# NikolausDemmel/rootba

Measured on NVIDIA H100. Metric: ms/LM-iter (linearize+QR+PCG) on BAL at 1/2/4/8 H100 vs CPU ref, lower is better.
Workload: dtype f32

## Files before the change

rootba_b200/csrc/kernels.cuh:

```cuda
#pragma once

#include <cooperative_groups.h>
#include <cuda_runtime.h>

#include <cfloat>
#include <cmath>
#include <cstdint>

#include "layout.hpp"

namespace rba {

template <class S> struct ST;
template <> struct ST<float> {
  using V2 = float2;
  using V4 = float4;
  __host__ __device__ static float eps_sqrt() { return 0.0031622776601683794f; }
  __host__ __device__ static float eps() { return 1e-5f; }
  __host__ __device__ static float tiny() { return FLT_MIN; }
};
template <> struct ST<double> {
  using V2 = double2;
  using V4 = double4;
  __host__ __device__ static double eps_sqrt() { return 1e-5; }
  __host__ __device__ static double eps() { return 1e-10; }
  __host__ __device__ static double tiny() { return DBL_MIN; }
};

__device__ __forceinline__ float2 mk2(float a, float b) { return make_float2(a, b); }
__device__ __forceinline__ double2 mk2(double a, double b) { return make_double2(a, b); }

struct KOpts {
  int use_valid_projections_only;
  int robust_norm;
  double huber;
  double jacobi_eps;
  int write_panel;
};

struct PcgState {
  double rho[2];
  double q0[2];
  double norm_b;
  double last_pq, last_alpha, last_zeta;
  int iter;
  int done;
  int term;
  int reason;
};

constexpr int NPART = 64;

template <class S>
struct DevPtrs {
  S* cams; S* lms;
  const TileInfo* tiles; int ntiles;
  const int* sorted_lm;
  const int* slot_cam; const int* slot_lm; const S* slot_xy; int nslots;
  S* panel;
  S* jp;
  S* q1u;
  S* q1d;
  S* jl;
  S* res;
  S* lmk;
  S* qtr;
  S* dmp;
  S* blk0;
  S* diag2; S* scaling; S* b; S* x; S* r; S* z; S* p; S* q; S* y; S* inc;
  S* blocks;
  S* jblocks;
  S* blocks0;
  S* b0;
  S* inv;
  S* yobs;
  S* partial;
  S* pblk;
  int nc;
  const uint8_t* cam_fixed;
  const S* prior_H;
  const int* pair_ptr;
  const int* pair_nbr;
  const S* pair_O;
  S* pair_ov;
  const int* lmp_slot;
  const S* lmp_mean;
  const S* lmp_L;
  S* lmp_Lg;
  const S* obs_W;
};
// ... 875 lines not shown
        V2* pk = ptile + (size_t)k * 32 + lane;
        const S nw00 = vc[0] ? -w0[0] : S(0), nw01 = vc[0] ? -w1[0] : S(0), nw02 = vc[0] ? -w2[0] : S(0);
        const S nw10 = vc[1] ? -w0[1] : S(0), nw11 = vc[1] ? -w1[1] : S(0), nw12 = vc[1] ? -w2[1] : S(0);
        const S* vp = sV + 9;
#pragma unroll 4
        for (int r = 3; r < nrows; ++r, vp += 3) {
          const S v0 = vp[0], v1 = vp[1], v2 = vp[2];
          pk[(size_t)(r - 3) * KP * 32] = mk2(nw00 * v0 + nw01 * v1 + nw02 * v2, nw10 * v0 + nw11 * v1 + nw12 * v2);
        }
#pragma unroll
        for (int v = 0; v < 2; ++v) {
          if (!vc[v]) continue;
#pragma unroll
          for (int q = 0; q < 2; ++q) {
            const int r = r2i[v] + q;
            if (r >= 3) {
              const S* vq = sV + 3 * r;
              const S val = (q == 0 ? a0[v] : a1[v]) - (w0[v] * vq[0] + w1[v] * vq[1] + w2[v] * vq[2]);
              S* dst = reinterpret_cast<S*>(pk + (size_t)(r - 3) * KP * 32) + v;
              *dst = val;
            }
          }
        }
      }
    }
#undef A_AT
    for (int e = lane; e < Wn; e += 32) sQ[28 * e + 27] = 0;
    __syncwarp();
    warp_copy_out(D.q1u + 28 * (size_t)T.slot_base, sQ, T.nvalid * n * 28, lane);
    __syncwarp();
  }
}


__host__ __device__ inline int stage2_need(int n, int G, int KP) {
  const int W = 32 / G, Wn = W * n;
  const int CS = (2 * G * KP) | 1;
  return 3 * W * CS + Wn * 9 + W * 20 + 8;
}

template <class S>
__device__ __forceinline__ void lm_prior_compress(const S* __restrict__ Lg, S sl, S (&C)[3][3], S (&c)[3]) {
  S M[6][4];
#pragma unroll
  for (int r = 0; r < 3; ++r) {
#pragma unroll
    for (int k = 0; k < 3; ++k) { M[r][k] = Lg[3 * r + k]; M[3 + r][k] = r == k ? sl : S(0); }
    M[r][3] = Lg[9 + r];
    M[3 + r][3] = 0;
  }
#pragma unroll
  for (int k = 0; k < 3; ++k)
#pragma unroll
    for (int m = k + 1; m < 6; ++m) {
      const Rot<S> gq = make_givens(M[k][k], M[m][k]);
#pragma unroll
      for (int cc = k; cc < 4; ++cc) rot_apply(gq, M[m][cc], M[k][cc]);
    }
#pragma unroll
  for (int r = 0; r < 3; ++r) {
#pragma unroll
    for (int k = 0; k < 3; ++k) C[r][k] = k >= r ? M[r][k] : S(0);
    c[r] = M[r][3];
  }
}

template <class S, bool PANEL, bool LMP = false>
__global__ void __launch_bounds__(128) k_stage2(DevPtrs<S> D, S lambda, Scratch<S> sc, int write_panel) {
  extern __shared__ __align__(16) unsigned char smem_raw[];
  using V2 = typename ST<S>::V2;
  const int wib = threadIdx.x >> 5, lane = threadIdx.x & 31;
  S* ws_smem = reinterpret_cast<S*>(smem_raw) + (size_t)wib * sc.smem_cap;
  for (int t = blockIdx.x * (blockDim.x >> 5) + wib; t < D.ntiles; t += gridDim.x * (blockDim.x >> 5)) {
    const TileInfo T = D.tiles[t];
    const int n = T.n, G = T.G, KP = T.KP, W = 32 / G, Wn = W * n;
    const int ncols = 9 * n;
    const int CS = (2 * G * KP) | 1;
    const int g = lane / G, j = lane - g * G;
    const bool active = g < T.nvalid;
    S* ws = scratch_ptr(sc, ws_smem, stage2_need(n, G, KP));
    S* sD = ws;
    S* sG = sD + 3 * W * CS;
    S* sRot = sG + Wn * 9;
    if (lane < T.nvalid) {
      S* lk = D.lmk + 24 * (size_t)(T.lm_base + lane);
      S Rw[3][3] = {{lk[0], lk[1], lk[2]}, {0, lk[3], lk[4]}, {0, 0, lk[5]}};
      S Dw[3][3] = {{0, 0, 0}, {0, 0, 0}, {0, 0, 0}};
      S rr[3] = {lk[6], lk[7], lk[8]}, dr[3] = {0, 0, 0};
      S* ro = sRot + 20 * lane;
      int lp = -1;
      if constexpr (LMP) lp = D.lmp_slot[T.lm_base + lane];
      if (lambda == S(0) && lp < 0) {
#pragma unroll
        for (int q = 0; q < 6; ++q) { ro[2 * q] = 1; ro[2 * q + 1] = 0; }
      } else {
        const S sl = sqrt(lambda);
        if (LMP && lp >= 0) lm_prior_compress(D.lmp_Lg + 12 * (size_t)lp, sl, Dw, dr);
        else { Dw[0][0] = sl; Dw[1][1] = sl; Dw[2][2] = sl; }
        int q = 0;
#pragma unroll
        for (int nn = 0; nn < 3; ++nn)
#pragma unroll
          for (int m = 0; m <= nn; ++m) {
            const int d = nn - m;
            const Rot<S> gq = make_givens(Rw[nn][nn], Dw[d][nn]);
            ro[2 * q] = gq.c; ro[2 * q + 1] = gq.s;
            ++q;
#pragma unroll
            for (int c = 0; c < 3; ++c) rot_apply(gq, Dw[d][c], Rw[nn][c]);
            rot_apply(gq, dr[d], rr[nn]);
          }
      }
      ro[12] = rr[0]; ro[13] = rr[1]; ro[14] = rr[2];
      ro[15] = dr[0]; ro[16] = dr[1]; ro[17] = dr[2];
      lk[9] = Rw[0][0]; lk[10] = Rw[0][1]; lk[11] = Rw[0][2]; lk[12] = Rw[1][1]; lk[13] = Rw[1][2]; lk[14] = Rw[2][2];
      lk[15] = rr[0]; lk[16] = rr[1]; lk[17] = rr[2];
    }
    __syncwarp();
    if (active) {
      Rot<S> rot[6];
      const S* ro = sRot + 20 * g;
#pragma unroll
      for (int q = 0; q < 6; ++q) { rot[q].c = ro[2 * q]; rot[q].s = ro[2 * q + 1]; }
      const S rr0 = ro[12], rr1 = ro[13], rr2 = ro[14];
      const S dr0 = ro[15], dr1 = ro[16], dr2 = ro[17];
      for (int i = j; i < n; i += G) {
        const size_t sl = (size_t)(T.slot_base + g * n + i);
        S q[28], jp[PANEL ? 4 : 20], dm[PANEL ? 28 : 4];
        load_rec<S, 28>(D.q1u + 28 * sl, q);
        S r0 = 0, r1 = 0;
        if constexpr (!PANEL) {
          load_rec<S, 20>(D.jp + 20 * sl, jp);
          r0 = D.res[2 * sl]; r1 = D.res[2 * sl + 1];
        }
        S* d0 = sD + (0 * W + g) * CS + 9 * i;
        S* d1 = sD + (1 * W + g) * CS + 9 * i;
        S* d2 = sD + (2 * W + g) * CS + 9 * i;
        S* go = sG + 9 * (g * n + i);
#pragma unroll
        for (int p = 0; p < 9; ++p) {
          S qv[3] = {q[p], q[9 + p], q[18 + p]}, dv[3] = {0, 0, 0};
          int qi = 0;
#pragma unroll
          for (int nn = 0; nn < 3; ++nn)
#pragma unroll
            for (int m = 0; m <= nn; ++m) rot_apply(rot[qi++], dv[nn - m], qv[nn]);
          q[p] = qv[0]; q[9 + p] = qv[1]; q[18 + p] = qv[2];
          d0[p] = dv[0]; d1[p] = dv[1]; d2[p] = dv[2];
          if constexpr (PANEL) {
            dm[p] = dv[0]; dm[9 + p] = dv[1]; dm[18 + p] = dv[2];
            go[p] = dv[0] * dr0 + dv[1] * dr1 + dv[2] * dr2;
          } else {
            go[p] = jp[p] * r0 + jp[9 + p] * r1 - (qv[0] * rr0 + qv[1] * rr1 + qv[2] * rr2);
          }
        }
        q[27] = 0;
        store_rec<S, 28>(D.q1d + 28 * sl, q);
        if constexpr (PANEL) {
          dm[27] = 0;
          store_rec<S, 28>(D.dmp + 28 * sl, dm);
        }
      }
    }
    __syncwarp();
    {
      const int nsl = T.nvalid * n;
      for (int e = lane; e < nsl * 9; e += 32) D.yobs[9 * (size_t)T.slot_base + e] = sG[e];
      if constexpr (!PANEL) {
        if (D.dmp)
          for (int e = lane; e < nsl * 28; e += 32) {
            const int sl = e / 28, k = e - 28 * sl, gg = sl / n, d = k / 9;
            D.dmp[28 * (size_t)T.slot_base + e] = k < 27 ? sD[(d * W + gg) * CS + 9 * (sl - gg * n) + (k - 9 * d)] : S(0);
          }
      }
      if (active && write_panel) {
        V2* ptile = reinterpret_cast<V2*>(D.panel + T.panel_off) + (size_t)(2 * n - 3) * KP * 32 + lane;
        for (int k = 0; k < KP; ++k) {
          const int c = 2 * j + 2 * G * k;
#pragma unroll
          for (int d = 0; d < 3; ++d) {
            const S* row = sD + (d * W + g) * CS;
            ptile[((size_t)d * KP + k) * 32] = mk2(c < ncols ? row[c] : S(0), c + 1 < ncols ? row[c + 1] : S(0));
          }
        }
      }
    }
    __syncwarp();
  }
}

template <class S, bool LMP = false>
__global__ void __launch_bounds__(128) k_sc_stage2(DevPtrs<S> D, S lambda) {
  const int wib = threadIdx.x >> 5, lane = threadIdx.x & 31;
  for (int t = blockIdx.x * (blockDim.x >> 5) + wib; t < D.ntiles; t += gridDim.x * (blockDim.x >> 5)) {
    const TileInfo T = D.tiles[t];
    const int n = T.n, G = T.G;
    const int g = lane / G, j = lane - g * G;
    const bool active = g < T.nvalid;
    const size_t slot0 = (size_t)(T.slot_base + g * n);
    S h[6] = {0, 0, 0, 0, 0, 0}, gv[3] = {0, 0, 0};
    if (active) {
      for (int i = j; i < n; i += G) {
        const S* jl = D.jl + 6 * (slot0 + i);
        const S r0 = D.res[2 * (slot0 + i)], r1 = D.res[2 * (slot0 + i) + 1];
        const S a0 = jl[0], a1 = jl[1], a2 = jl[2], b0 = jl[3], b1 = jl[4], b2 = jl[5];
        h[0] += a0 * a0 + b0 * b0; h[1] += a0 * a1 + b0 * b1; h[2] += a0 * a2 + b0 * b2;
        h[3] += a1 * a1 + b1 * b1; h[4] += a1 * a2 + b1 * b2; h[5] += a2 * a2 + b2 * b2;
        gv[0] += a0 * r0 + b0 * r1; gv[1] += a1 * r0 + b1 * r1; gv[2] += a2 * r0 + b2 * r1;
      }
    }
#pragma unroll
    for (int k = 0; k < 6; ++k) h[k] = group_sum(h[k], G);
#pragma unroll
    for (int k = 0; k < 3; ++k) gv[k] = group_sum(gv[k], G);
    if constexpr (LMP) {
      const int lp = D.lmp_slot[T.lm_base + g];
      if (lp >= 0) {
        const S* pg = D.lmp_Lg + 12 * (size_t)lp;
#pragma unroll
        for (int r = 0; r < 3; ++r) {
          const S a0 = pg[3 * r], a1 = pg[3 * r + 1], a2 = pg[3 * r + 2], gr = pg[9 + r];
          h[0] += a0 * a0; h[1] += a0 * a1; h[2] += a0 * a2; h[3] += a1 * a1; h[4] += a1 * a2; h[5] += a2 * a2;
          gv[0] += a0 * gr; gv[1] += a1 * gr; gv[2] += a2 * gr;
        }
      }
    }
    h[0] += lambda; h[3] += lambda; h[5] += lambda;
    const S r00 = sqrt(h[0]);
    const S r01 = h[1] / r00, r02 = h[2] / r00;
    const S r11 = sqrt(h[3] - r01 * r01);
    const S r12 = (h[4] - r01 * r02) / r11;
    const S r22 = sqrt(h[5] - r02 * r02 - r12 * r12);
    const S rr0 = gv[0] / r00;
    const S rr1 = (gv[1] - r01 * rr0) / r11;
    const S rr2 = (gv[2] - r02 * rr0 - r12 * rr1) / r22;
    if (active && j == 0) {
      S* lk = D.lmk + 24 * (size_t)(T.lm_base + g);
      lk[9] = r00; lk[10] = r01; lk[11] = r02; lk[12] = r11; lk[13] = r12; lk[14] = r22;
      lk[15] = rr0; lk[16] = rr1; lk[17] = rr2;
    }
    if (active) {
      for (int i = j; i < n; i += G) {
        const size_t sl = slot0 + i;
        S jp[20], q[28];
        load_rec<S, 20>(D.jp + 20 * sl, jp);
        const S* jl = D.jl + 6 * sl;
        const S a0 = jl[0], a1 = jl[1], a2 = jl[2], b0 = jl[3], b1 = jl[4], b2 = jl[5];
        const S r0 = D.res[2 * sl], r1 = D.res[2 * sl + 1];
        S* go = D.yobs + 9 * sl;
#pragma unroll
        for (int p = 0; p < 9; ++p) {
          const S t0 = a0 * jp[p] + b0 * jp[9 + p], t1 = a1 * jp[p] + b1 * jp[9 + p], t2 = a2 * jp[p] + b2 * jp[9 + p];
          const S c0 = t0 / r00;
          const S c1 = (t1 - r01 * c0) / r11;
          const S c2 = (t2 - r02 * c0 - r12 * c1) / r22;
          q[p] = c0; q[9 + p] = c1; q[18 + p] = c2;
          go[p] = jp[p] * r0 + jp[9 + p] * r1 - (c0 * rr0 + c1 * rr1 + c2 * rr2);
        }
        q[27] = 0;
        store_rec<S, 28>(D.q1d + 28 * sl, q);
      }
    }
  }
}

template <class S>
__global__ void __launch_bounds__(128) k_matvec_implicit(DevPtrs<S> D, int tile_begin, const S* __restrict__ xvec, const int* done, int pdl,
                                                          int e0_only = 0) {
  if (done && *reinterpret_cast<const volatile int*>(done)) return;
  if (pdl) asm volatile("griddepcontrol.wait;" ::: "memory");
  if (done && *done) return;
  if (pdl) asm volatile("griddepcontrol.launch_dependents;" ::: "memory");
  const int wib = threadIdx.x >> 5, lane = threadIdx.x & 31;
  for (int t = tile_begin + blockIdx.x * (blockDim.x >> 5) + wib; t < D.ntiles; t += gridDim.x * (blockDim.x >> 5)) {
    const TileInfo T = D.tiles[t];
    const int n = T.n, G = T.G;
    const int g = lane / G, j = lane - g * G;
    const bool active = g < T.nvalid;
    const size_t sl0 = (size_t)(T.slot_base + g * n);
    S u0 = 0, u1 = 0, u2 = 0;
    if (active) {
      for (int i = j; i < n; i += G) {
        const size_t sl = sl0 + i;
        S q[28];
        load_rec<S, 28>(D.q1d + 28 * sl, q);
        const S* xc = xvec + 9 * (size_t)D.slot_cam[sl];
#pragma unroll
        for (int p = 0; p < 9; ++p) {
          const S xv = xc[p];
          u0 += q[p] * xv; u1 += q[9 + p] * xv; u2 += q[18 + p] * xv;
        }
      }
    }
    u0 = group_sum(u0, G); u1 = group_sum(u1, G); u2 = group_sum(u2, G);
    if (active) {
      for (int i = j; i < n; i += G) {
        const size_t sl = sl0 + i;
        S q[28], jp[20];
        load_rec<S, 28>(D.q1d + 28 * sl, q);
        load_rec<S, 20>(D.jp + 20 * sl, jp);
        const S* xc = xvec + 9 * (size_t)D.slot_cam[sl];
        S t0 = 0, t1 = 0;
#pragma unroll
        for (int p = 0; p < 9; ++p) {
          const S xv = xc[p];
          t0 += jp[p] * xv; t1 += jp[9 + p] * xv;
        }
        S* yo = D.yobs + 9 * sl;
#pragma unroll
        for (int p = 0; p < 9; ++p) {
          const S e0 = q[p] * u0 + q[9 + p] * u1 + q[18 + p] * u2;
          yo[p] = e0_only ? e0 : (jp[p] * t0 + jp[9 + p] * t1) - e0;
        }
      }
    }
  }
}

template <class S, int MODE>
__global__ void __launch_bounds__(128) k_precond_partial(const S* __restrict__ recA, const S* __restrict__ recB,
                                                          const int* __restrict__ slots, const ReduceItem* __restrict__ items,
                                                          int nitems, S* __restrict__ pblk) {
  const int it = blockIdx.x * blockDim.x + threadIdx.x;
  if (it >= nitems) return;
  const ReduceItem I = items[it];
  S acc[45];
#pragma unroll
  for (int k = 0; k < 45; ++k) acc[k] = 0;
  for (int e = I.begin; e < I.end; ++e) {
    const size_t sl = (size_t)slots[e];
    if constexpr (MODE == 3) {
      S v[48];
      load_rec<S, 48>(recA + 48 * sl, v);
#pragma unroll
      for (int k = 0; k < 45; ++k) acc[k] += v[k];
    } else if constexpr (MODE == 2) {
      S v[28];
      load_rec<S, 28>(recA + 28 * sl, v);
      int k = 0;
#pragma unroll
      for (int a = 0; a < 9; ++a)
#pragma unroll
        for (int b = a; b < 9; ++b) acc[k++] += v[a] * v[b] + v[9 + a] * v[9 + b] + v[18 + a] * v[18 + b];
    } else {
      S v[20], w[MODE == 1 ? 28 : 4];
      load_rec<S, 20>(recA + 20 * sl, v);
      if constexpr (MODE == 1) load_rec<S, 28>(recB + 28 * sl, w);
      int k = 0;
#pragma unroll
      for (int a = 0; a < 9; ++a)
#pragma unroll
        for (int b = a; b < 9; ++b) {
          S sacc = v[a] * v[b] + v[9 + a] * v[9 + b];
          if constexpr (MODE == 1) sacc -= w[a] * w[b] + w[9 + a] * w[9 + b] + w[18 + a] * w[18 + b];
          acc[k++] += sacc;
        }
    }
  }
  S* o = pblk + 48 * (size_t)it;
#pragma unroll
  for (int k = 0; k < 45; ++k) o[k] = acc[k];
}

template <class S>
__global__ void k_precond_final(const S* __restrict__ pblk, const int* __restrict__ cam_item_ptr, int nc,
                                const S* __restrict__ addend, S* __restrict__ blocks) {
  const int i = blockIdx.x * blockDim.x + threadIdx.x;
  if (i >= 45 * nc) return;
  const int cam = i / 45, k = i - 45 * cam;
  S s = 0;
  for (int it = cam_item_ptr[cam]; it < cam_item_ptr[cam + 1]; ++it) s += pblk[48 * (size_t)it + k];
  int a = 0, rem = k;
  while (rem >= 9 - a) { rem -= 9 - a; ++a; }
  const int b = a + rem;
  if (addend) s += addend[81 * (size_t)cam + 9 * a + b];
  blocks[81 * (size_t)cam + 9 * a + b] = s;
  blocks[81 * (size_t)cam + 9 * b + a] = s;
}

template <class S>
__global__ void __launch_bounds__(128) k_panel_grad_blocks(DevPtrs<S> D, int want_blocks, TileOrder to) {
  using V2 = typename ST<S>::V2;
  const int wib = threadIdx.x >> 5, lane = threadIdx.x & 31;
  for (int idx = blockIdx.x * (blockDim.x >> 5) + wib;; idx += gridDim.x * (blockDim.x >> 5)) {
    const int t = tile_at(to, idx, D.ntiles);
    if (t < 0) break;
    const TileInfo T = D.tiles[t];
    const int n = T.n, G = T.G, KP = T.KP;
    const int lg = 31 - __clz(G);
    const int nobs = T.nvalid * n;
    const int nrows = 2 * n - 3;
    const V2* __restrict__ ptile = reinterpret_cast<const V2*>(D.panel + T.panel_off);
    const size_t rstride = (size_t)KP * 32;
    for (int e = lane; e < nobs; e += 32) {
      const int g = e / n, i = e - g * n;
      const int c0 = 9 * i;
      const bool odd = c0 & 1;
      const int p0 = c0 >> 1;
      int off[5];
#pragma unroll
      for (int q = 0; q < 5; ++q) {
        const int p = p0 + q;
        off[q] = (p >> lg) * 32 + g * G + (p & (G - 1));
      }
      const S* __restrict__ tq = D.qtr + 2 * (size_t)(T.slot_base + g * n) + 3;
      S acc[45], gacc[9];
#pragma unroll
      for (int k = 0; k < 45; ++k) acc[k] = 0;
#pragma unroll
      for (int k = 0; k < 9; ++k) gacc[k] = 0;
#pragma unroll 2
      for (int r = 0; r < nrows; ++r) {
        const V2* pr = ptile + (size_t)r * rstride;
        V2 a[5];
#pragma unroll
        for (int q = 0; q < 5; ++q) a[q] = __ldg(pr + off[q]);
        const S tr = __ldg(tq + r);
        const S el[10] = {a[0].x, a[0].y, a[1].x, a[1].y, a[2].x, a[2].y, a[3].x, a[3].y, a[4].x, a[4].y};
        S v[9];
#pragma unroll
        for (int k = 0; k < 9; ++k) v[k] = odd ? el[k + 1] : el[k];
#pragma unroll
        for (int k = 0; k < 9; ++k) gacc[k] += v[k] * tr;
        if (want_blocks) {
          int k = 0;
#pragma unroll
          for (int x = 0; x < 9; ++x)
#pragma unroll
            for (int y = x; y < 9; ++y) acc[k++] += v[x] * v[y];
        }
      }
      const size_t sl = (size_t)(T.slot_base + e);
#pragma unroll
      for (int k = 0; k < 9; ++k) D.yobs[9 * sl + k] = gacc[k];
      if (want_blocks) {
        S o[48];
#pragma unroll
        for (int k = 0; k < 45; ++k) o[k] = acc[k];
        o[45] = o[46] = o[47] = 0;
        store_rec<S, 48>(D.blk0 + 48 * sl, o);
      }
    }
  }
}

template <class S>
__global__ void __launch_bounds__(64) k_precond_invert(const S* __restrict__ src, S lambda, int nc,
                                                        S* __restrict__ blocks_out, S* __restrict__ inv,
                                                        const uint8_t* __restrict__ cam_fixed, S* __restrict__ b,
                                                        const S* __restrict__ prior_H = nullptr, const S* __restrict__ prior_g = nullptr) {
  const int cam = blockIdx.x * blockDim.x + threadIdx.x;
  if (cam >= nc) return;
  const unsigned fm = cam_fixed ? fixed_entry_mask(cam_fixed[cam]) : 0u;
  S A[9][9];
#pragma unroll
  for (int r = 0; r < 9; ++r)
#pragma unroll
    for (int c = 0; c < 9; ++c) A[r][c] = src[81 * (size_t)cam + 9 * r + c];
  if (prior_H)
#pragma unroll
    for (int r = 0; r < 9; ++r)
#pragma unroll
      for (int c = 0; c < 9; ++c) A[r][c] += prior_H[81 * (size_t)cam + 9 * r + c];
  if (prior_g)
#pragma unroll
    for (int d = 0; d < 9; ++d) b[9 * (size_t)cam + d] += prior_g[9 * (size_t)cam + d];
#pragma unroll
  for (int d = 0; d < 9; ++d) A[d][d] += lambda;
  if (blocks_out)
#pragma unroll
    for (int r = 0; r < 9; ++r)
#pragma unroll
      for (int c = 0; c < 9; ++c) blocks_out[81 * (size_t)cam + 9 * r + c] = A[r][c];
  if (fm) {
#pragma unroll
    for (int r = 0; r < 9; ++r)
#pragma unroll
      for (int c = 0; c < 9; ++c)
        if (((fm >> r) | (fm >> c)) & 1u) A[r][c] = (r == c) ? S(1) : S(0);
#pragma unroll
    for (int d = 0; d < 9; ++d)
      if ((fm >> d) & 1u) b[9 * (size_t)cam + d] = S(0);
  }
#pragma unroll
  for (int jj = 0; jj < 9; ++jj) {
    S sdiag = A[jj][jj];
#pragma unroll
    for (int k = 0; k < jj; ++k) sdiag -= A[jj][k] * A[jj][k];
    const S d = sqrt(sdiag);
    A[jj][jj] = d;
#pragma unroll
    for (int i = jj + 1; i < 9; ++i) {
      S t = A[jj][i];
#pragma unroll
      for (int k = 0; k < jj; ++k) t -= A[i][k] * A[jj][k];
      A[i][jj] = t / d;
    }
  }
  S Li[9][9];
#pragma unroll
  for (int c = 0; c < 9; ++c) {
#pragma unroll
    for (int r = 0; r < 9; ++r) {
      if (r < c) Li[r][c] = 0;
      else {
        S t = (r == c) ? S(1) : S(0);
#pragma unroll
        for (int k = 0; k < 9; ++k) if (k >= c && k < r) t -= A[r][k] * Li[k][c];
        Li[r][c] = t / A[r][r];
      }
    }
  }
  if (fm)
#pragma unroll
    for (int d = 0; d < 9; ++d)
      if ((fm >> d) & 1u) Li[d][d] = S(0);
  S* out = inv + 81 * (size_t)cam;
#pragma unroll
  for (int r = 0; r < 9; ++r)
#pragma unroll
    for (int c = r; c < 9; ++c) {
      S t = 0;
#pragma unroll
      for (int k = 0; k < 9; ++k) if (k >= c) t += Li[k][r] * Li[k][c];
// ... 1469 lines not shown
```

rootba_b200/csrc/solver.cu:

```cuda
#include <cuda_runtime.h>
#include <dlfcn.h>

#include <cstdio>
#include <cstdlib>
#include <cstring>
#include <chrono>
#include <array>
#include <limits>
#include <memory>
#include <string>
#include <utility>
#include <vector>

#include "../../include/rootba_b200.h"
#include "../host/bal_io_fast.hpp"
#include "kernels.cuh"
#include "covariance.cuh"
#include "assembled.cuh"
#include "groups.cuh"
#include "nccl_dyn.hpp"

namespace rba {

thread_local std::string g_err;
// ... 1027 lines not shown
  int compute_error(rba_residual_info* out) override {
    int rc = compute_error_enqueue(); if (rc) return rc;
    if (error_enqueued) CU(cudaStreamSynchronize(stream));
    return compute_error_finish(out);
  }

  int linearize_enqueue() {
    lin_l0 = launches;
    const int n_pairs = pprior.n, n_groups = grp.n;
    int rc = start(ev_stage1); if (rc) return rc;
    CU(cudaMemsetAsync(d_flags, 0, 4 * sizeof(int), stream));
    auto kn = D.obs_W ? k_jp_norms<S, true> : k_jp_norms<S>;
    kn<<<grid_for(L.nslots, 256, 8), 256, 0, stream>>>(D, ko, d_flags);
    ++launches;
    rc = camera_reduce(d_csr_obs_slots, d_csr_obs_items, n_obs_items, d_csr_obs_item_ptr, D.diag2); if (rc) return rc;
    if (cprior.on) {
      k_prior_linearize<S><<<(nc + 127) / 128, 128, 0, stream>>>(D.cams, cprior.mean.get(), cprior.L.get(), nc, D.diag2, cprior.A.get(), cprior.r.get());
      ++launches;
    }
    if (n_pairs > 0) {
      k_pair_linearize<S><<<(n_pairs + 127) / 128, 128, 0, stream>>>(D.cams, pprior.ij.get(), pprior.mean.get(), pprior.L.get(), n_pairs, pprior.A.get(), pprior.r.get());
      k_pair_diag2<S><<<(nc + 127) / 128, 128, 0, stream>>>(pprior.A.get(), pprior.ptr.get(), pprior.item.get(), nc, D.diag2);
      launches += 2;
    }
    if (n_groups) {
      k_group_sum_diag2<S><<<n_groups, GROUP_THREADS, 0, stream>>>(D.diag2, groups());
      ++launches;
    }
    k_scaling<S><<<(9 * nc + 255) / 256, 256, 0, stream>>>(D.diag2, D.scaling, 9 * nc, (S)ko.jacobi_eps);
    const bool lmp = D.lmp_slot != nullptr;
    auto k1 = opt.use_householder_marginalization ? (lmp ? k_linearize_qr<S, false, true> : k_linearize_qr<S, false>)
                                                  : (lmp ? k_linearize_qr<S, true, true> : k_linearize_qr<S, true>);
    if (D.obs_W)
      k1 = opt.use_householder_marginalization ? (lmp ? k_linearize_qr<S, false, true, true> : k_linearize_qr<S, false, false, true>)
                                               : (lmp ? k_linearize_qr<S, true, true, true> : k_linearize_qr<S, true, false, true>);
    k1<<<tile_grid(k1_max_blocks), TILE_WARPS * 32, k1_smem, stream>>>(D, ko, k1_sc, d_flags, order_k1);
    launches += 2;
    if (opt.preconditioner_type == 0 || opt.solver_type == 2) {
      rc = precond_blocks(0, D.jblocks, nullptr, true); if (rc) return rc;
    }
    const bool jac = opt.preconditioner_type == 0 || opt.solver_type == 2;
    if (cprior.on) {
      k_prior_scale<S><<<(nc + 127) / 128, 128, 0, stream>>>(cprior.A.get(), cprior.r.get(), D.scaling, nc, cprior.H.get(), cprior.g.get(), jac ? D.jblocks : nullptr);
      ++launches;
    }
    if (n_pairs > 0) {
      k_pair_scale<S><<<(n_pairs + 127) / 128, 128, 0, stream>>>(pprior.A.get(), pprior.ij.get(), D.scaling, n_pairs);
      k_pair_accum<S><<<(nc + 127) / 128, 128, 0, stream>>>(pprior.A.get(), pprior.r.get(), pprior.ptr.get(), pprior.item.get(), nc, (int)cprior.on,
                                                            cprior.H.get(), cprior.g.get(), jac ? D.jblocks : nullptr, pprior.O.get());
      launches += 2;
    }
    if (panel_form()) {
      const int want_blocks = opt.preconditioner_type == 1 ? 1 : 0;
      k_panel_grad_blocks<S><<<tile_grid(sm_count * 8), TILE_WARPS * 32, 0, stream>>>(D, want_blocks, order_kp);
      ++launches;
      rc = camera_reduce(d_csr_obs_slots, d_csr_obs_items, n_obs_items, d_csr_obs_item_ptr, D.b0, nullptr, false); if (rc) return rc;
      if (want_blocks) { rc = precond_blocks(3, D.blocks0, nullptr, false); if (rc) return rc; }
    }
    rc = allreduce_scalars(0); if (rc) return rc;
    CU(cudaMemcpyAsync(h_res->linearize_flags, d_flags, sizeof(h_res->linearize_flags), cudaMemcpyDeviceToHost, stream));
    rc = stop(ev_stage1); if (rc) return rc;
    linearized = true;
    new_linearization_point = true;
    su_valid = s_valid = false;
    damping_valid = false;
    have_inc = false;
    return RBA_OK;
  }
  int linearize_finish() {
    CU(cudaGetLastError());
    tm.stage1_time = elapsed(ev_stage1);
    tm.kernel_launches = launches - lin_l0;
    if (h_res->linearize_flags[1]) { linearized = false; g_err = "a peer rank did not take part in a cross-shard reduction in time (peer-memory exchange timed out)"; return RBA_ERR_NCCL; }
    if (h_res->linearize_flags[0]) { linearized = false; return RBA_NUMERICAL_FAILURE; }
    return RBA_OK;
  }
  int linearize() override {
    int rc = linearize_enqueue(); if (rc) return rc;
    CU(cudaStreamSynchronize(stream));
    return linearize_finish();
  }

  int precond_blocks(int mode, S* dst, const S* addend, bool reduce_ranks) {
    const int g = (n_pb_items + 127) / 128;
    switch (mode) {
      case 0: k_precond_partial<S, 0><<<g, 128, 0, stream>>>(D.jp, (const S*)nullptr, d_csr_obs_slots, d_pb_items, n_pb_items, D.pblk); break;
      case 1: k_precond_partial<S, 1><<<g, 128, 0, stream>>>(D.jp, D.q1d, d_csr_obs_slots, d_pb_items, n_pb_items, D.pblk); break;
      case 2: k_precond_partial<S, 2><<<g, 128, 0, stream>>>(D.dmp, (const S*)nullptr, d_csr_obs_slots, d_pb_items, n_pb_items, D.pblk); break;
      default: k_precond_partial<S, 3><<<g, 128, 0, stream>>>(D.blk0, (const S*)nullptr, d_csr_obs_slots, d_pb_items, n_pb_items, D.pblk); break;
    }
    k_precond_final<S><<<(45 * nc + 255) / 256, 256, 0, stream>>>(D.pblk, d_pb_item_ptr, nc, addend, dst);
    launches += 2;
    return reduce_ranks ? allreduce(dst, (size_t)81 * nc) : RBA_OK;
  }

  enum class Handover {
    Assembled,
    Partials,
    Counter,
    Peer,
    Nccl,
  };
  Handover handover() const {
    if (s_valid) return Handover::Assembled;
    if (grp.n) return opt.nranks > 1 ? Handover::Nccl : Handover::Counter;
    if (opt.nranks > 1) return peer_ok ? Handover::Peer : Handover::Nccl;
    const bool vec_cached = 9 * ((nc + pcg_cluster - 1) / pcg_cluster) <= VEC_THREADS * VEC_EPT;
    return pcg_partials && vec_cached && opt.solver_type != 2 ? Handover::Partials : Handover::Counter;
  }
  int apply_operator(const S* xvec, Handover h, bool in_solve, int e0_only = 0) {
    const int* done = in_solve ? &d_state->done : nullptr;
    const bool pdl = in_solve;
    ++tm.matvec_launches;
    if (h == Handover::Assembled) {
      const bool p = pdl && !s_fresh;
      s_fresh = false;
      return launch_ex(k_rcs_spmv<S>, spmv_grid, SPMV_CLASSES * 32, 0, p, 1, (const SpmvChunk*)d_spmv_chunks, (const int*)d_spmv_chunk_ptr,
                       (const int*)d_asm_col, (const S*)d_asm_S, xvec, D.y, done, (int)p);
    }
    if (panels) {
      if (L.n_items_large > 0) {
        k_matvec_large<S, K4_WARPS, KPMAX><<<grid_for(L.n_items_large, K4_WARPS, 4), K4_WARPS * 32, k4_smem_small, stream>>>(
            D, d_items, 0, L.n_items_large, L.k4_scratch_per_warp, xvec, done);
        ++launches;
      }
      const bool p = pdl && L.n_items_large == 0;
      if (n_dealt > L.n_items_large)
        TRY(launch_ex(k_matvec_small_tma<S, K4_WARPS, K4_NS, K4_STAGE>, tma_grid, K4_WARPS * 32, K4_SMEM_TMA, p, 1, D, (const MatvecItem*)d_items, L.n_items_large, n_dealt, xvec, done, (int)p));
    } else {
      const int ntl = (int)L.tiles.size();
      const bool p = pdl && imp_tile_split == ntl;
      if (imp_tile_split > 0)
        TRY(launch_ex((k_matvec_implicit_tma<S, IMP_WARPS, IMP_MAXSLOTS, IMP_NS>), imp_grid, IMP_WARPS * 32, imp_smem, p, 1, D, imp_tile_split, xvec, done, (int)p, e0_only));
      if (imp_tile_split < ntl)
        TRY(launch_ex(k_matvec_implicit<S>, (ntl - imp_tile_split + TILE_WARPS - 1) / TILE_WARPS, TILE_WARPS * 32, 0, false, 1, D, imp_tile_split, xvec, done, 0, e0_only));
    }
    const int grid = grid_for(n_op_items, 8, 8);
    if (h == Handover::Partials)
      return launch_ex(k_cam_reduce<S>, grid, 256, 0, pdl, 1, (const S*)D.yobs, op_slots, op_items, n_op_items, D.partial, done, (int)pdl);
    if (h == Handover::Peer) ++ar_seq;
    if (h == Handover::Nccl) CU(cudaMemsetAsync(D.y, 0, (size_t)9 * nc * sizeof(S), stream));
    auto kern = h == Handover::Peer ? k_cam_reduce_final<S, true> : k_cam_reduce_final<S, false>;
    TRY(launch_ex(kern, grid, 256, 0, pdl, 1, (const S*)D.yobs, op_slots, op_items, n_op_items, op_item_ptr, D.partial, d_cam_cnt, D.y, done, (int)pdl, pc, ar_seq, nc));
    return h == Handover::Nccl ? allreduce(D.y, (size_t)9 * nc) : RBA_OK;
  }
  int matvec_launch(const S* xvec, bool clear_y) {
    const Handover h = handover() == Handover::Assembled ? Handover::Assembled : Handover::Counter;
    if (clear_y && h == Handover::Counter) CU(cudaMemsetAsync(D.y, 0, (size_t)9 * nc * sizeof(S), stream));
    return apply_operator(xvec, h, false);
  }
  int pcg_vec(int i, int mode, bool pdl, int is_last, S lambda, bool fused_ar = false, bool from_partials = false) {
    PeerComm c = pc;
    if (!fused_ar) c.nranks = 1;
    DevPtrs<S> Dv = D;
    if (grp.n) {
      Dv.y = grp.y.get(); Dv.prior_H = nullptr; Dv.pair_ov = nullptr;
    }
    if (Dv.pair_ov && mode != 3) TRY(pair_ov(mode == 2 ? D.x : D.p, pdl));
    auto kern = Dv.pair_ov ? k_pcg_vec<S, true, true> : Dv.prior_H ? k_pcg_vec<S, true> : k_pcg_vec<S, false>;
    return launch_ex(kern, pcg_cluster, VEC_THREADS, 0, pdl, pcg_cluster, Dv, d_state, lambda, i, mode, (double)opt.eta,
                     (int)opt.min_linear_solver_iterations, is_last, (int)pdl, c, ar_seq, from_partials ? op_item_ptr : (const int*)nullptr, d_prog);
  }
  int pair_ov(const S* v, bool pdl) {
    return launch_ex(k_pair_ov<S>, (9 * nc + 255) / 256, 256, 0, pdl, 1, D, (const PcgState*)d_state, v);
  }
  int pcg_step(int i, int mode, int is_last, S lambda, Handover h) {
    const S* v = mode == 2 ? D.x : D.p;
    if (grp.n) {
      TRY(group_expand(v, grp.ve.get(), true));
      v = grp.ve.get();
    }
    TRY(apply_operator(v, h, true));
// ... 966 lines not shown
```

Before: 5.550.

## Coalesce precond partial and panel block stores via warp-cooperative shared staging

Rewrites k_precond_partial so each warp handles one reduce item. The warp cooperatively loads the item's records into shared memory with vector loads, and each lane then accumulates one or two of the 45 block entries instead of one thread holding all 45. k_panel_grad_blocks now stages per-lane gradients and 45-entry blocks through shared memory so the global stores are coalesced. Stage2 in PANEL mode writes dmp through the existing shared-tile coalesced path instead of per-thread strided record stores, and prefetches the first q1u record before the rotation setup. The cost is extra shared memory and warp syncs, plus a static assumption that PB_SEG_LEN is at most 32.

```diff
diff --git a/rootba_b200/csrc/kernels.cuh b/rootba_b200/csrc/kernels.cuh
--- a/rootba_b200/csrc/kernels.cuh
+++ b/rootba_b200/csrc/kernels.cuh
@@ -6,6 +6,7 @@
 #include <cfloat>
 #include <cmath>
 #include <cstdint>
+#include <type_traits>
 
 #include "layout.hpp"
 
@@ -1047,6 +1048,8 @@
     S* sD = ws;
     S* sG = sD + 3 * W * CS;
     S* sRot = sG + Wn * 9;
+    S rec[28];
+    if (PANEL && active && j < n) load_rec<S, 28>(D.q1u + 28 * (size_t)(T.slot_base + g * n + j), rec);
     if (lane < T.nvalid) {
       S* lk = D.lmk + 24 * (size_t)(T.lm_base + lane);
       S Rw[3][3] = {{lk[0], lk[1], lk[2]}, {0, lk[3], lk[4]}, {0, 0, lk[5]}};
@@ -1091,8 +1094,8 @@
       const S dr0 = ro[15], dr1 = ro[16], dr2 = ro[17];
       for (int i = j; i < n; i += G) {
         const size_t sl = (size_t)(T.slot_base + g * n + i);
-        S q[28], jp[PANEL ? 4 : 20], dm[PANEL ? 28 : 4];
-        load_rec<S, 28>(D.q1u + 28 * sl, q);
+        S jp[PANEL ? 4 : 20];
+        if (!PANEL || i != j) load_rec<S, 28>(D.q1u + 28 * sl, rec);
         S r0 = 0, r1 = 0;
         if constexpr (!PANEL) {
           load_rec<S, 20>(D.jp + 20 * sl, jp);
@@ -1104,40 +1107,33 @@
         S* go = sG + 9 * (g * n + i);
 #pragma unroll
         for (int p = 0; p < 9; ++p) {
-          S qv[3] = {q[p], q[9 + p], q[18 + p]}, dv[3] = {0, 0, 0};
+          S qv[3] = {rec[p], rec[9 + p], rec[18 + p]}, dv[3] = {0, 0, 0};
           int qi = 0;
 #pragma unroll
           for (int nn = 0; nn < 3; ++nn)
 #pragma unroll
             for (int m = 0; m <= nn; ++m) rot_apply(rot[qi++], dv[nn - m], qv[nn]);
-          q[p] = qv[0]; q[9 + p] = qv[1]; q[18 + p] = qv[2];
+          rec[p] = qv[0]; rec[9 + p] = qv[1]; rec[18 + p] = qv[2];
           d0[p] = dv[0]; d1[p] = dv[1]; d2[p] = dv[2];
           if constexpr (PANEL) {
-            dm[p] = dv[0]; dm[9 + p] = dv[1]; dm[18 + p] = dv[2];
             go[p] = dv[0] * dr0 + dv[1] * dr1 + dv[2] * dr2;
           } else {
             go[p] = jp[p] * r0 + jp[9 + p] * r1 - (qv[0] * rr0 + qv[1] * rr1 + qv[2] * rr2);
           }
         }
-        q[27] = 0;
-        store_rec<S, 28>(D.q1d + 28 * sl, q);
-        if constexpr (PANEL) {
-          dm[27] = 0;
-          store_rec<S, 28>(D.dmp + 28 * sl, dm);
-        }
+        rec[27] = 0;
+        store_rec<S, 28>(D.q1d + 28 * sl, rec);
       }
     }
     __syncwarp();
     {
       const int nsl = T.nvalid * n;
       for (int e = lane; e < nsl * 9; e += 32) D.yobs[9 * (size_t)T.slot_base + e] = sG[e];
-      if constexpr (!PANEL) {
-        if (D.dmp)
-          for (int e = lane; e < nsl * 28; e += 32) {
-            const int sl = e / 28, k = e - 28 * sl, gg = sl / n, d = k / 9;
-            D.dmp[28 * (size_t)T.slot_base + e] = k < 27 ? sD[(d * W + gg) * CS + 9 * (sl - gg * n) + (k - 9 * d)] : S(0);
-          }
-      }
+      if (D.dmp)
+        for (int e = lane; e < nsl * 28; e += 32) {
+          const int sl = e / 28, k = e - 28 * sl, gg = sl / n, d = k / 9;
+          D.dmp[28 * (size_t)T.slot_base + e] = k < 27 ? sD[(d * W + gg) * CS + 9 * (sl - gg * n) + (k - 9 * d)] : S(0);
+        }
       if (active && write_panel) {
         V2* ptile = reinterpret_cast<V2*>(D.panel + T.panel_off) + (size_t)(2 * n - 3) * KP * 32 + lane;
         for (int k = 0; k < KP; ++k) {
@@ -1282,49 +1278,78 @@
   }
 }
 
+template <int MODE> struct PrecondRec {
+  static constexpr int A = MODE == 3 ? 48 : MODE == 2 ? 28 : 20;
+  static constexpr int B = MODE == 1 ? 28 : 0;
+};
+constexpr int PB_WARPS = 4;
+static_assert(PB_SEG_LEN <= 32, "k_precond_partial stages one slot index per lane");
+
 template <class S, int MODE>
-__global__ void __launch_bounds__(128) k_precond_partial(const S* __restrict__ recA, const S* __restrict__ recB,
-                                                          const int* __restrict__ slots, const ReduceItem* __restrict__ items,
-                                                          int nitems, S* __restrict__ pblk) {
-  const int it = blockIdx.x * blockDim.x + threadIdx.x;
+__device__ __forceinline__ S precond_term(const S* v, const S* w, int k, int a, int b) {
+  if constexpr (MODE == 3) {
+    return v[k];
+  } else if constexpr (MODE == 2) {
+    return v[a] * v[b] + v[9 + a] * v[9 + b] + v[18 + a] * v[18 + b];
+  } else {
+    S sacc = v[a] * v[b] + v[9 + a] * v[9 + b];
+    if constexpr (MODE == 1) sacc -= w[a] * w[b] + w[9 + a] * w[9 + b] + w[18 + a] * w[18 + b];
+    return sacc;
+  }
+}
+
+template <class S, int MODE>
+__global__ void __launch_bounds__(PB_WARPS * 32) k_precond_partial(const S* __restrict__ recA, const S* __restrict__ recB,
+                                                                    const int* __restrict__ slots, const ReduceItem* __restrict__ items,
+                                                                    int nitems, S* __restrict__ pblk) {
+  using R = PrecondRec<MODE>;
+  using V = typename std::conditional<sizeof(S) == 4, float4, double2>::type;
+  constexpr int PER_V = 16 / sizeof(S);
+  constexpr int NA = R::A / PER_V, NB = R::B / PER_V;
+  constexpr int NV = (PB_SEG_LEN * (NA + NB) + 31) / 32;
+  __shared__ __align__(16) S srec[PB_WARPS][PB_SEG_LEN * (R::A + R::B)];
+  __shared__ int sidx[PB_WARPS][PB_SEG_LEN];
+  const int wib = threadIdx.x >> 5, lane = threadIdx.x & 31;
+  const int it = blockIdx.x * PB_WARPS + wib;
   if (it >= nitems) return;
   const ReduceItem I = items[it];
-  S acc[45];
-#pragma unroll
-  for (int k = 0; k < 45; ++k) acc[k] = 0;
-  for (int e = I.begin; e < I.end; ++e) {
-    const size_t sl = (size_t)slots[e];
-    if constexpr (MODE == 3) {
-      S v[48];
-      load_rec<S, 48>(recA + 48 * sl, v);
-#pragma unroll
-      for (int k = 0; k < 45; ++k) acc[k] += v[k];
-    } else if constexpr (MODE == 2) {
-      S v[28];
-      load_rec<S, 28>(recA + 28 * sl, v);
-      int k = 0;
-#pragma unroll
-      for (int a = 0; a < 9; ++a)
-#pragma unroll
-        for (int b = a; b < 9; ++b) acc[k++] += v[a] * v[b] + v[9 + a] * v[9 + b] + v[18 + a] * v[18 + b];
-    } else {
-      S v[20], w[MODE == 1 ? 28 : 4];
-      load_rec<S, 20>(recA + 20 * sl, v);
-      if constexpr (MODE == 1) load_rec<S, 28>(recB + 28 * sl, w);
-      int k = 0;
-#pragma unroll
-      for (int a = 0; a < 9; ++a)
-#pragma unroll
-        for (int b = a; b < 9; ++b) {
-          S sacc = v[a] * v[b] + v[9 + a] * v[9 + b];
-          if constexpr (MODE == 1) sacc -= w[a] * w[b] + w[9 + a] * w[9 + b] + w[18 + a] * w[18 + b];
-          acc[k++] += sacc;
-        }
-    }
+  const int cnt = I.end - I.begin;
+  if (lane < cnt) sidx[wib][lane] = __ldg(slots + I.begin + lane);
+  __syncwarp();
+  S* sa = srec[wib];
+  S* sb = sa + PB_SEG_LEN * R::A;
+  V buf[NV];
+#pragma unroll
+  for (int t = 0; t < NV; ++t) {
+    const int q = lane + 32 * t;
+    if (q < cnt * NA) {
+      const int e = q / NA;
+      buf[t] = __ldg(reinterpret_cast<const V*>(recA + (size_t)R::A * sidx[wib][e]) + (q - NA * e));
+    } else if (NB && q < PB_SEG_LEN * NA + cnt * NB && q >= PB_SEG_LEN * NA) {
+      const int qb = q - PB_SEG_LEN * NA, e = qb / (NB ? NB : 1);
+      buf[t] = __ldg(reinterpret_cast<const V*>(recB + (size_t)R::B * sidx[wib][e]) + (qb - NB * e));
+    }
+  }
+  V* sv = reinterpret_cast<V*>(sa);
+#pragma unroll
+  for (int t = 0; t < NV; ++t)
+    if (lane + 32 * t < PB_SEG_LEN * (NA + NB)) sv[lane + 32 * t] = buf[t];
+  __syncwarp();
+  const int k0 = lane, k1 = lane + 32;
+  int a0 = 0, r0 = k0, a1 = 0, r1 = k1 < 45 ? k1 : 0;
+  while (r0 >= 9 - a0) { r0 -= 9 - a0; ++a0; }
+  while (r1 >= 9 - a1) { r1 -= 9 - a1; ++a1; }
+  const int b0 = a0 + r0, b1 = a1 + r1;
+  S acc0 = 0, acc1 = 0;
+  for (int e = 0; e < cnt; ++e) {
+    const S* v = sa + R::A * e;
+    const S* w = sb + R::B * e;
+    acc0 += precond_term<S, MODE>(v, w, k0, a0, b0);
+    if (k1 < 45) acc1 += precond_term<S, MODE>(v, w, k1, a1, b1);
   }
   S* o = pblk + 48 * (size_t)it;
-#pragma unroll
-  for (int k = 0; k < 45; ++k) o[k] = acc[k];
+  o[k0] = acc0;
+  if (k1 < 45) o[k1] = acc1;
 }
 
 template <class S>
@@ -1346,7 +1371,12 @@
 template <class S>
 __global__ void __launch_bounds__(128) k_panel_grad_blocks(DevPtrs<S> D, int want_blocks, TileOrder to) {
   using V2 = typename ST<S>::V2;
+  constexpr int HALF = 24, HS = HALF + 1;
+  __shared__ S sg_all[4][32 * 9];
+  __shared__ S sb_all[4][32 * HS];
   const int wib = threadIdx.x >> 5, lane = threadIdx.x & 31;
+  S* sg = sg_all[wib];
+  S* sb = sb_all[wib];
   for (int idx = blockIdx.x * (blockDim.x >> 5) + wib;; idx += gridDim.x * (blockDim.x >> 5)) {
     const int t = tile_at(to, idx, D.ntiles);
     if (t < 0) break;
@@ -1357,54 +1387,66 @@
     const int nrows = 2 * n - 3;
     const V2* __restrict__ ptile = reinterpret_cast<const V2*>(D.panel + T.panel_off);
     const size_t rstride = (size_t)KP * 32;
-    for (int e = lane; e < nobs; e += 32) {
-      const int g = e / n, i = e - g * n;
-      const int c0 = 9 * i;
-      const bool odd = c0 & 1;
-      const int p0 = c0 >> 1;
-      int off[5];
-#pragma unroll
-      for (int q = 0; q < 5; ++q) {
-        const int p = p0 + q;
-        off[q] = (p >> lg) * 32 + g * G + (p & (G - 1));
-      }
-      const S* __restrict__ tq = D.qtr + 2 * (size_t)(T.slot_base + g * n) + 3;
+    for (int e0 = 0; e0 < nobs; e0 += 32) {
+      const int e = e0 + lane, cnt = min(32, nobs - e0);
       S acc[45], gacc[9];
 #pragma unroll
       for (int k = 0; k < 45; ++k) acc[k] = 0;
 #pragma unroll
       for (int k = 0; k < 9; ++k) gacc[k] = 0;
+      if (e < nobs) {
+        const int g = e / n, i = e - g * n;
+        const int c0 = 9 * i;
+        const bool odd = c0 & 1;
+        const int p0 = c0 >> 1;
+        int off[5];
+#pragma unroll
+        for (int q = 0; q < 5; ++q) {
+          const int p = p0 + q;
+          off[q] = (p >> lg) * 32 + g * G + (p & (G - 1));
+        }
+        const S* __restrict__ tq = D.qtr + 2 * (size_t)(T.slot_base + g * n) + 3;
 #pragma unroll 2
-      for (int r = 0; r < nrows; ++r) {
-        const V2* pr = ptile + (size_t)r * rstride;
-        V2 a[5];
-#pragma unroll
-        for (int q = 0; q < 5; ++q) a[q] = __ldg(pr + off[q]);
-        const S tr = __ldg(tq + r);
-        const S el[10] = {a[0].x, a[0].y, a[1].x, a[1].y, a[2].x, a[2].y, a[3].x, a[3].y, a[4].x, a[4].y};
-        S v[9];
-#pragma unroll
-        for (int k = 0; k < 9; ++k) v[k] = odd ? el[k + 1] : el[k];
-#pragma unroll
-        for (int k = 0; k < 9; ++k) gacc[k] += v[k] * tr;
-        if (want_blocks) {
-          int k = 0;
-#pragma unroll
-          for (int x = 0; x < 9; ++x)
-#pragma unroll
-            for (int y = x; y < 9; ++y) acc[k++] += v[x] * v[y];
+        for (int r = 0; r < nrows; ++r) {
+          const V2* pr = ptile + (size_t)r * rstride;
+          V2 a[5];
+#pragma unroll
+          for (int q = 0; q < 5; ++q) a[q] = __ldg(pr + off[q]);
+          const S tr = __ldg(tq + r);
+          const S el[10] = {a[0].x, a[0].y, a[1].x, a[1].y, a[2].x, a[2].y, a[3].x, a[3].y, a[4].x, a[4].y};
+          S v[9];
+#pragma unroll
+          for (int k = 0; k < 9; ++k) v[k] = odd ? el[k + 1] : el[k];
+#pragma unroll
+          for (int k = 0; k < 9; ++k) gacc[k] += v[k] * tr;
+          if (want_blocks) {
+            int k = 0;
+#pragma unroll
+            for (int x = 0; x < 9; ++x)
+#pragma unroll
+              for (int y = x; y < 9; ++y) acc[k++] += v[x] * v[y];
+          }
         }
       }
-      const size_t sl = (size_t)(T.slot_base + e);
-#pragma unroll
-      for (int k = 0; k < 9; ++k) D.yobs[9 * sl + k] = gacc[k];
+      const size_t sl0 = (size_t)(T.slot_base + e0);
+#pragma unroll
+      for (int k = 0; k < 9; ++k) sg[9 * lane + k] = gacc[k];
+      __syncwarp();
+      for (int q = lane; q < 9 * cnt; q += 32) D.yobs[9 * sl0 + q] = sg[q];
       if (want_blocks) {
-        S o[48];
-#pragma unroll
-        for (int k = 0; k < 45; ++k) o[k] = acc[k];
-        o[45] = o[46] = o[47] = 0;
-        store_rec<S, 48>(D.blk0 + 48 * sl, o);
-      }
+#pragma unroll
+        for (int h = 0; h < 2; ++h) {
+#pragma unroll
+          for (int k = 0; k < HALF; ++k) sb[HS * lane + k] = HALF * h + k < 45 ? acc[HALF * h + k] : S(0);
+          __syncwarp();
+          for (int q = lane; q < HALF * cnt; q += 32) {
+            const int r = q / HALF, k = q - HALF * r;
+            D.blk0[48 * (sl0 + r) + HALF * h + k] = sb[HS * r + k];
+          }
+          __syncwarp();
+        }
+      }
+      __syncwarp();
     }
   }
 }
diff --git a/rootba_b200/csrc/solver.cu b/rootba_b200/csrc/solver.cu
--- a/rootba_b200/csrc/solver.cu
+++ b/rootba_b200/csrc/solver.cu
@@ -1133,12 +1133,12 @@
   }
 
   int precond_blocks(int mode, S* dst, const S* addend, bool reduce_ranks) {
-    const int g = (n_pb_items + 127) / 128;
+    const int g = (n_pb_items + PB_WARPS - 1) / PB_WARPS;
     switch (mode) {
-      case 0: k_precond_partial<S, 0><<<g, 128, 0, stream>>>(D.jp, (const S*)nullptr, d_csr_obs_slots, d_pb_items, n_pb_items, D.pblk); break;
-      case 1: k_precond_partial<S, 1><<<g, 128, 0, stream>>>(D.jp, D.q1d, d_csr_obs_slots, d_pb_items, n_pb_items, D.pblk); break;
-      case 2: k_precond_partial<S, 2><<<g, 128, 0, stream>>>(D.dmp, (const S*)nullptr, d_csr_obs_slots, d_pb_items, n_pb_items, D.pblk); break;
-      default: k_precond_partial<S, 3><<<g, 128, 0, stream>>>(D.blk0, (const S*)nullptr, d_csr_obs_slots, d_pb_items, n_pb_items, D.pblk); break;
+      case 0: k_precond_partial<S, 0><<<g, PB_WARPS * 32, 0, stream>>>(D.jp, (const S*)nullptr, d_csr_obs_slots, d_pb_items, n_pb_items, D.pblk); break;
+      case 1: k_precond_partial<S, 1><<<g, PB_WARPS * 32, 0, stream>>>(D.jp, D.q1d, d_csr_obs_slots, d_pb_items, n_pb_items, D.pblk); break;
+      case 2: k_precond_partial<S, 2><<<g, PB_WARPS * 32, 0, stream>>>(D.dmp, (const S*)nullptr, d_csr_obs_slots, d_pb_items, n_pb_items, D.pblk); break;
+      default: k_precond_partial<S, 3><<<g, PB_WARPS * 32, 0, stream>>>(D.blk0, (const S*)nullptr, d_csr_obs_slots, d_pb_items, n_pb_items, D.pblk); break;
     }
     k_precond_final<S><<<(45 * nc + 255) / 256, 256, 0, stream>>>(D.pblk, d_pb_item_ptr, nc, addend, dst);
     launches += 2;
```

Result: faster. 5.427 (median of 6 runs) (-2.2%).
